# TimGyger/GPBoost

Measured on AMD Instinct MI355X. Metric: neg-log-lik + grad evals/sec, n=100k Vecchia m=30, higher is better.
Workload: dtype f64; 1 GPU; vecchia_gaussian_exact_lbfgs_unit; n=100000, num_neighbors=30, cov_function=exponential, ordering=random, parallelism=rows1

## Files before the change

gpboost_amd/csrc/vecchia_rows16.hip:

```cpp
#include <hip/hip_runtime.h>

#include <algorithm>
#include <type_traits>

#include "common.h"
#include "cov.h"
#include "kernels.h"

namespace gpb_amd {
namespace {

constexpr int kD3 = 3;

__device__ __forceinline__ void lds_sync() { asm volatile("s_waitcnt lgkmcnt(0)" ::: "memory"); }
__device__ __forceinline__ void cfence() { asm volatile("" ::: "memory"); }

template <int CTRL>
__device__ __forceinline__ double dpp32x2(double v) {
  const int lo = __builtin_amdgcn_mov_dpp(__double2loint(v), CTRL, 0xF, 0xF, true);
  const int hi = __builtin_amdgcn_mov_dpp(__double2hiint(v), CTRL, 0xF, 0xF, true);
  return __hiloint2double(hi, lo);
}

template <int L>
__device__ __forceinline__ double bcast16(double v) {
  const long b = __builtin_amdgcn_mov_dpp(__builtin_bit_cast(long, v), 0x150 + L, 0xF, 0xF, true);
  return __builtin_bit_cast(double, b);
}

template <int L, bool NOP = false>
__device__ __forceinline__ void fmac_bcast16(double& acc, double src, double mul) {
  if constexpr (NOP)
    asm volatile("s_nop 1\n\tv_fmac_f64_dpp %0, %1, %2 row_newbcast:%3 row_mask:0xf bank_mask:0xf"
                 : "+v"(acc)
                 : "v"(src), "v"(mul), "n"(L));
  else
    asm volatile("v_fmac_f64_dpp %0, %1, %2 row_newbcast:%3 row_mask:0xf bank_mask:0xf"
                 : "+v"(acc)
                 : "v"(src), "v"(mul), "n"(L));
}

__device__ __forceinline__ unsigned lds_addr(const double* p) {
  return (unsigned)(size_t)(const __attribute__((address_space(3))) double*)p;
}

template <int C>
__device__ __forceinline__ void lds_read_split2(double& a, double& b, unsigned up_a, unsigned up_b, unsigned lo_a,
                                                unsigned lo_b) {
  constexpr unsigned m16 = (0xFFFFu << C) & 0xFFFFu;
  constexpr unsigned long mask = m16 | m16 << 16;
  constexpr int CB = C + 16;
  unsigned long saved;
  asm volatile(
      "ds_read_b64 %0, %3 offset:%7\n\t"
      "ds_read_b64 %1, %4 offset:%8\n\t"
      "s_mov_b64 %2, exec\n\t"
      "s_and_b32 exec_lo, exec_lo, %11\n\t"
      "s_and_b32 exec_hi, exec_hi, %11\n\t"
      "ds_read_b64 %0, %5 offset:%9\n\t"
      "ds_read_b64 %1, %6 offset:%10\n\t"
      "s_mov_b64 exec, %2"
      : "=&v"(a), "=&v"(b), "=&s"(saved)
      : "v"(up_a), "v"(up_b), "v"(lo_a), "v"(lo_b), "n"(C * (C + 1) / 2 * 8), "n"(CB * (CB + 1) / 2 * 8), "n"(C * 8),
        "n"(CB * 8), "n"(mask)
      : "memory", "scc");
}

__device__ __forceinline__ double sum16(double v) {
  v += dpp32x2<0xB1>(v);
  v += dpp32x2<0x4E>(v);
  v += dpp32x2<0x141>(v);
  v += dpp32x2<0x140>(v);
  return v;
}

__device__ __forceinline__ double recip(double x) {
  double r = __builtin_amdgcn_rcp(x);
  r = fma(r, fma(-x, r, 1.), r);
  return fma(r, fma(-x, r, 1.), r);
}

template <int B, int E, class F>
__device__ __forceinline__ void sfor(F&& f) {
  if constexpr (B < E) {
    f(std::integral_constant<int, B>{});
    sfor<B + 1, E>(f);
  }
}

__device__ __forceinline__ int tri(int x) { return x * (x + 1) / 2; }

constexpr int kK = 32, kMK = 30;
constexpr int kPacked = kK * (kK + 1) / 2;

template <int CS>
constexpr int problem_doubles() { return kPacked + 48 * CS; }

typedef double v2d __attribute__((ext_vector_type(2)));


template <int ND>
__device__ __forceinline__ void load_points(const VecchiaRowsArgs& a, int d, int irow, int h, bool rv0, bool rv1,
                                            int nb0, int nb1, double (&xi)[ND], double (&x0)[ND], double (&x1)[ND]) {
#pragma unroll
  for (int q = 0; q < ND; ++q) {
    xi[q] = (q < d) ? a.X[(size_t)irow * d + q] : 0.;
    x0[q] = (q < d && rv0) ? a.X[(size_t)nb0 * d + q] : 0.;
    x1[q] = (q < d && rv1) ? a.X[(size_t)nb1 * d + q] : 0.;
  }
}

template <int ND>
__device__ __forceinline__ void pad_points(int h, bool rv0, bool rv1, const double (&xi)[ND], double (&x0)[ND],
                                           double (&x1)[ND]) {
  const int v1 = h + 16;
  const bool own1 = v1 == kMK;
#pragma unroll
  for (int q = 0; q < ND; ++q) x1[q] = own1 ? xi[q] : x1[q];
  x0[0] = rv0 ? x0[0] : 1e30 * (h + 1);
  x1[0] = (rv1 || own1) ? x1[0] : 1e30 * (v1 + 1);
}

template <int ND>
__device__ __forceinline__ void put_points(double* nbx, int h, const double (&x0)[ND], const double (&x1)[ND]) {
  const int v1 = h + 16;
#pragma unroll
  for (int q = 0; q < ND; ++q) {
    nbx[h * ND + q] = x0[q];
    nbx[(h + 31) * ND + q] = x0[q];
    if (v1 <= kMK) nbx[v1 * ND + q] = x1[q];
  }
}

template <int ND>
__device__ __forceinline__ double sq_dist(const double (&x)[ND], const double* xp) {
  double s = 0.;
#pragma unroll
  for (int q = 0; q < ND; ++q) {
    const double t = x[q] - xp[q];
    s += t * t;
  }
  return s;
}

constexpr int kDistRecs = 15 * 16;
static_assert(2 * kDistRecs == kRows16DistDoubles, "record layout");

template <int COV, int DIM, bool STORED>
__device__ __forceinline__ void rows16_body(const VecchiaRowsArgs& a) {
  constexpr int ND = DIM > 0 ? DIM : kD3;
  constexpr int CS = STORED ? 2 : ND;
  constexpr int PD = problem_doubles<CS>();
  static_assert(PD % 2 == 0, "16-byte aligned problems");
  extern __shared__ __attribute__((aligned(16))) double smem[];
  const int lane = threadIdx.x;
  const int g = lane >> 4;
  double* Cp = smem + g * PD;
  double* nbx = Cp + kPacked;
  const double var = a.var, phi = a.phi;
  const double cdiag = var * a.diag_mult + a.diag_add;
  const double delta = cdiag - var;
  const bool want_like = a.Y != nullptr;
  [[maybe_unused]] const int d = DIM > 0 ? DIM : a.d;

  double* acc = smem + 4 * PD + g * kVecchiaSums;
  if ((lane & 15) < kVecchiaSums) acc[lane & 15] = 0.;
  const int total = a.r1 - a.r0;
  const ExpCoef ek = ExpCoef::scalar();
  const int nsets = (total + 3) / 4, G = gridDim.x, w = blockIdx.x;
  const int R = (nsets + G - 1) / G, E = nsets - (R - 1) * G;
  int last_set = (R - 1) * G + w;
  if (a.sched == 1) {
    const long lo = (long)w * E / G, hi = (long)(w + 1) * E / G;
    last_set = hi > lo ? (R - 1) * G + (int)lo : nsets;
  }
  auto set_at = [&](int it) { return it + 1 < R ? it * G + w : last_set; };
  v2d rr[STORED ? 15 : 1];
  int pnb0 = 0, pnb1 = 0;
  auto prefetch = [&](int set) {
    if constexpr (STORED) {
      const int h = lane & 15;
      const int i = a.r0 + set * 4 + g;
      const bool active = i < a.r1;
      const int k = active ? min(i, a.m) : 0;
      pnb0 = h < k ? a.nbr[(size_t)(i - a.row_base) * a.m + h] : 0;
      pnb1 = h + 16 < k ? a.nbr[(size_t)(i - a.row_base) * a.m + h + 16] : 0;
      const v2d* rp = reinterpret_cast<const v2d*>(a.R) + (size_t)((active ? i : a.r0) - a.row_base) * kDistRecs + h;
#pragma unroll
      for (int q = 0; q < 15; ++q) rr[q] = rp[q * 16];
    }
  };
  if (set_at(0) < nsets) prefetch(set_at(0));
  for (int it = 0; it < R; ++it) {
    const int set = set_at(it);
    if (set >= nsets) break;
    const int base = set * 4;
    int h = lane & 15;
    asm volatile("" : "+v"(h));
    const int v1 = h + 16;
    const int i = a.r0 + base + g;
    const bool active = i < a.r1;
    const int k = active ? min(i, a.m) : 0;
    const bool rv0 = h < k, rv1 = v1 < k;
    const int irow = active ? i : a.r0;

    int nb0, nb1;
    double xi[ND], x0[ND], x1[ND];
    if constexpr (STORED) {
      nb0 = pnb0;
      nb1 = pnb1;
    } else {
      nb0 = rv0 ? a.nbr[(size_t)(i - a.row_base) * a.m + h] : 0;
      nb1 = rv1 ? a.nbr[(size_t)(i - a.row_base) * a.m + v1] : 0;
      load_points<ND>(a, d, irow, h, rv0, rv1, nb0, nb1, xi, x0, x1);
    }
    const double yi = want_like ? a.Y[irow] : 0.;
    double y0s = (want_like && rv0) ? a.Y[nb0] : 0.;
    double y1s = (want_like && rv1) ? a.Y[nb1] : 0.;
    if constexpr (!STORED) pad_points<ND>(h, rv0, rv1, xi, x0, x1);
    cfence();
    if constexpr (!STORED) put_points<ND>(nbx, h, x0, x1);
    Cp[tri(h) + h] = rv0 ? cdiag : 1.;
    Cp[tri(v1) + v1] = rv1 ? cdiag : 1.;
    lds_sync();

    double w0[15], w1[15];
    {
      const int b0 = tri(h) + h, b1 = tri(v1) + v1;
#pragma unroll
      for (int dl = 1; dl <= 15; ++dl) {
        double cv, dcv;
        if constexpr (STORED) cov_dcov_r<COV>(rr[dl - 1].x, var, phi, cv, dcv, ek);
        else cov_dcov_sq<COV>(sq_dist<ND>(x0, nbx + (h + dl) * CS), var, phi, cv, dcv, ek);
        Cp[b0 + h * dl + dl * (dl + 1) / 2] = cv;
        w0[dl - 1] = dcv;
      }
#pragma unroll
      for (int dl = 1; dl <= 15; ++dl) {
        double cv, dcv;
        if constexpr (STORED) cov_dcov_r<COV>(rr[dl - 1].y, var, phi, cv, dcv, ek);
        else cov_dcov_sq<COV>(sq_dist<ND>(x1, nbx + (v1 + dl) * CS), var, phi, cv, dcv, ek);
        const int pos = (v1 + dl <= kMK) ? b1 + v1 * dl + dl * (dl + 1) / 2 : b1 + dl - 31;
        Cp[pos] = cv;
        w1[dl - 1] = dcv;
      }
    }
    lds_sync();
    Cp[tri(kMK + 1) + h] = y0s;
    if (v1 < kMK) Cp[tri(kMK + 1) + v1] = y1s;
    else if (v1 == kMK) Cp[tri(kMK + 1) + kMK] = 0.;
    lds_sync();

    double r0[kK], r1[kK];
    {
      const unsigned lo0 = lds_addr(Cp + tri(h)), up0 = lds_addr(Cp + h);
      const unsigned lo1 = lds_addr(Cp + tri(v1)), up1 = lds_addr(Cp + v1);
      r0[0] = Cp[tri(h)];
#pragma unroll
      for (int c = 16; c < kK; ++c) r0[c] = Cp[tri(c) + h];
#pragma unroll
      for (int c = 0; c <= 16; ++c) r1[c] = Cp[tri(v1) + c];
      sfor<1, 16>([&](auto C) {
        constexpr int c = decltype(C)::value;
        double &p0 = r0[c], &p1 = r1[c + 16];
        lds_read_split2<c>(p0, p1, up0, up1, lo0, lo1);
      });
      sfor<0, 3>([&](auto Q) {
        constexpr int q = 1 + 5 * decltype(Q)::value;
        double &a0 = r0[q], &a1 = r0[q + 1], &a2 = r0[q + 2], &a3 = r0[q + 3], &a4 = r0[q + 4];
        double &b0 = r1[q + 16], &b1 = r1[q + 17], &b2 = r1[q + 18], &b3 = r1[q + 19], &b4 = r1[q + 20];
        if constexpr (q == 1)
          asm volatile("s_waitcnt lgkmcnt(0)" : "+v"(a0), "+v"(a1), "+v"(a2), "+v"(a3), "+v"(a4), "+v"(b0), "+v"(b1), "+v"(b2), "+v"(b3), "+v"(b4));
        else
          asm volatile("" : "+v"(a0), "+v"(a1), "+v"(a2), "+v"(a3), "+v"(a4), "+v"(b0), "+v"(b1), "+v"(b2), "+v"(b3), "+v"(b4));
      });
    }
    double c0, c1, dc0, dc1;
    cfence();
    {
      v2d* st = reinterpret_cast<v2d*>(__builtin_assume_aligned(nbx, 16)) + 2 * h;
      st[0] = v2d{r0[kMK], rv1 ? r1[kMK] : 0.};
      st[1] = v2d{y0s, y1s};
    }
#pragma unroll
    for (int dl = 1; dl <= 15; ++dl) {
      Cp[(dl - 1) * kK + h] = w0[dl - 1];
      Cp[(dl - 1) * kK + v1] = w1[dl - 1];
    }

    double dg0 = 1., dg1 = 1.;
    auto pivot = [&](auto J, double& m0, double& m1) {
      constexpr int j = decltype(J)::value;
      constexpr int jl = j & 15;
      const double piv = bcast16<jl>(j >= 16 ? r1[j] : r0[j]);
      const double rinv = recip(piv);
      const bool own = h == jl;
      const double f1 = r1[j] * rinv;
      if constexpr (j >= 16) {
        m0 = 0.;
        m1 = -(own ? 0. : f1);
        dg1 = own ? piv : dg1;
      } else {
        const double f0 = r0[j] * rinv;
        m0 = -(own ? 0. : f0);
        m1 = -f1;
        dg0 = own ? piv : dg0;
      }
    };
    sfor<0, kMK>([&](auto J) {
      constexpr int j = decltype(J)::value;
      constexpr bool jhi = j >= 16;
      double nf0, nf1;
      pivot(J, nf0, nf1);
      constexpr int cA = jhi ? 0 : 16;
      sfor<j + 1, kK>([&](auto C) {
        constexpr int c = decltype(C)::value;
        constexpr bool first = c == j + 1;
        const double& src = c >= 16 ? r1[j] : r0[j];
        if constexpr (c < cA) fmac_bcast16<c & 15, first>(r0[c], src, nf0);
        fmac_bcast16<c & 15, first && !(c < cA)>(r1[c], src, nf1);
      });
      sfor<j + 1, kK>([&](auto C) {
        constexpr int c = decltype(C)::value;
        double &p0 = r0[c], &p1 = r1[c];
        if constexpr (c < cA) asm volatile("" : "+v"(p0), "+v"(p1));
        else asm volatile("" : "+v"(p1));
      });
      if constexpr (!jhi) r0[j] = nf0;
    });
    {
      const double i1 = recip(dg1);
      const double na = rv1 ? -(r1[kMK] * i1) : 0., nw = rv1 ? -(r1[kMK + 1] * i1) : 0.;
      sfor<16, kMK>([&](auto C) {
        constexpr int c = decltype(C)::value;
        fmac_bcast16<c & 15, c == 16>(r0[kMK], na, r0[c]);
        fmac_bcast16<c & 15, c == 16>(r0[kMK + 1], nw, r0[c]);
      });
      sfor<0, 16>([&](auto J) {
        constexpr int j = decltype(J)::value;
        fmac_bcast16<j, true>(r0[kMK], r0[kMK], r0[j]);
        fmac_bcast16<j>(r0[kMK + 1], r0[kMK + 1], r0[j]);
      });
    }
    if constexpr (STORED) {
      cfence();
      const int nxt = it + 1 < R ? set_at(it + 1) : nsets;
      prefetch(nxt < nsets ? nxt : set);
    }
    {
      lds_sync();
      const v2d* st = reinterpret_cast<const v2d*>(__builtin_assume_aligned(nbx, 16)) + 2 * h;
      const v2d s0 = st[0], s1 = st[1];
      c0 = s0.x;
      c1 = s0.y;
      y0s = s1.x;
      y1s = s1.y;
      dc0 = Cp[h <= 14 ? h * kK + kMK : 14 * kK + 15];
      dc1 = h <= 13 ? Cp[(13 - h) * kK + v1] : 0.;
    }
    const double i0 = recip(dg0), i1 = recip(dg1);
    const double a0 = rv0 ? r0[kMK] * i0 : 0., w0v = rv0 ? r0[kMK + 1] * i0 : 0.;
    const double a1 = rv1 ? r1[kMK] * i1 : 0., w1v = rv1 ? r1[kMK + 1] * i1 : 0.;
    if (active && a.B_out != nullptr) {
      double* Bo = a.B_out + (size_t)(i - a.row_base) * a.m;
      if (h < a.m) Bo[h] = rv0 ? -a0 : 0.;
      if (v1 < a.m) Bo[v1] = rv1 ? -a1 : 0.;
    }

    double tA, tV;
    {
      v2d* av2 = reinterpret_cast<v2d*>(__builtin_assume_aligned(nbx, 16));
      cfence();
      av2[h] = v2d{a0, w0v};
      if (v1 <= kMK) av2[v1] = v2d{a1, w1v};
      av2[h + 31] = v2d{a0, w0v};
      lds_sync();
      double s10 = 0., s20 = 0., s11 = 0., s21 = 0.;
#pragma unroll
      for (int dl = 1; dl <= 15; ++dl) {
        const double wa = Cp[(dl - 1) * kK + h], wb = Cp[(dl - 1) * kK + v1];
        const v2d pa = av2[h + dl], pb = av2[v1 + dl];
        s10 = fma(wa, pa.x, s10);
        s20 = fma(wa, pa.y, s20);
        s11 = fma(wb, pb.x, s11);
        s21 = fma(wb, pb.y, s21);
      }
      tA = 2. * (a0 * s10 + a1 * s11);
      tV = w0v * s10 + a0 * s20 + w1v * s11 + a1 * s21;
    }

    const double ac = sum16(a0 * c0 + a1 * c1);
    const double ay = sum16(a0 * y0s + a1 * y1s);
    const double aa = sum16(a0 * a0 + a1 * a1);
    const double avv = sum16(a0 * w0v + a1 * w1v);
    const double dca = sum16(dc0 * a0 + dc1 * a1);
    const double dcv = sum16(dc0 * w0v + dc1 * w1v);
    const double ta = sum16(tA);
    const double tv = sum16(tV);
    const double D = var + a.d_nugget - ac;
    const double Dinv = 1. / D;
    if (active && h == 0 && a.Dinv_out != nullptr) a.Dinv_out[i - a.row_base] = Dinv;
    if (want_like && active && h == 0) {
      const double By = yi - ay;
      const double u = By * Dinv;
      const double dD_var = var - delta * aa - ac;
      const double uk_var = -delta * avv;
      const double dD_rng = -(2. * dca - ta);
      const double uk_rng = -(dcv - tv);
      acc[0] += log(D);
      acc[1] += By * u;
      acc[2] += uk_var * u - 0.5 * u * u * dD_var;
      acc[3] += uk_rng * u - 0.5 * u * u * dD_rng;
      acc[4] += Dinv * dD_var;
      acc[5] += Dinv * dD_rng;
    }
  }
  if (!want_like) return;
  __syncthreads();
  const double* red = smem + 4 * PD;
  if (lane < kVecchiaSums) {
    const double v = ((red[lane] + red[kVecchiaSums + lane]) + red[2 * kVecchiaSums + lane]) + red[3 * kVecchiaSums + lane];
    a.block_sums[(size_t)blockIdx.x * kVecchiaSums + lane] = v;
  }
}

template <int COV, int DIM>
__global__ void __launch_bounds__(64) __attribute__((amdgpu_waves_per_eu(2, 2))) vecchia_rows16_kernel(VecchiaRowsArgs a) {
  rows16_body<COV, DIM, false>(a);
}

template <int COV>
__global__ void __launch_bounds__(64) __attribute__((amdgpu_waves_per_eu(2, 2))) vecchia_rows16d_kernel(VecchiaRowsArgs a) {
  rows16_body<COV, 2, true>(a);
}

template <int DIM>
__global__ void __launch_bounds__(64) vecchia_rows16_dist_kernel(VecchiaRowsArgs a, double* R) {
  constexpr int ND = DIM > 0 ? DIM : kD3;
  extern __shared__ __attribute__((aligned(16))) double smem[];
  const int lane = threadIdx.x;
  const int g = lane >> 4, h = lane & 15, v1 = h + 16;
  double* nbx = smem + g * 48 * ND;
  const int d = DIM > 0 ? DIM : a.d;
  const int nsets = (a.r1 - a.r0 + 3) / 4;
  for (int set = blockIdx.x; set < nsets; set += gridDim.x) {
    const int i = a.r0 + set * 4 + g;
    const bool active = i < a.r1;
    const int k = active ? min(i, a.m) : 0;
    const bool rv0 = h < k, rv1 = v1 < k;
    const int irow = active ? i : a.r0;
    const int nb0 = rv0 ? a.nbr[(size_t)(i - a.row_base) * a.m + h] : 0;
    const int nb1 = rv1 ? a.nbr[(size_t)(i - a.row_base) * a.m + v1] : 0;
    double xi[ND], x0[ND], x1[ND];
    load_points<ND>(a, d, irow, h, rv0, rv1, nb0, nb1, xi, x0, x1);
    pad_points<ND>(h, rv0, rv1, xi, x0, x1);
    cfence();
    put_points<ND>(nbx, h, x0, x1);
    lds_sync();
    v2d* out = reinterpret_cast<v2d*>(R) + (size_t)(irow - a.row_base) * kDistRecs + h;
#pragma unroll
    for (int dl = 1; dl <= 15; ++dl) {
      const double ra = sqrt_nonneg(sq_dist<ND>(x0, nbx + (h + dl) * ND));
      const double rb = sqrt_nonneg(sq_dist<ND>(x1, nbx + (v1 + dl) * ND));
      if (active) out[(dl - 1) * 16] = v2d{ra, rb};
    }
  }
}

constexpr int kMaxGrid = 2048;

template <auto KERN>
int launch16_at(size_t lds, const VecchiaRowsArgs& a, hipStream_t s) {
  static int cap = 0;
  if (cap == 0) {
    int dev = 0, cus = 0, per_cu = 0;
    HIP_CHECK(hipGetDevice(&dev));
    HIP_CHECK(hipDeviceGetAttribute(&cus, hipDeviceAttributeMultiprocessorCount, dev));
    HIP_CHECK(hipOccupancyMaxActiveBlocksPerMultiprocessor(&per_cu, KERN, 64, lds));
    cap = std::max(1, std::min(per_cu * cus, kMaxGrid));
  }
  const int need = (a.r1 - a.r0 + 3) / 4;
  int blocks = std::min(need, cap);
  if (a.sched == 2) {
    const int rounds = (need + blocks - 1) / blocks;
    blocks = (need + rounds - 1) / rounds;
  }
  hipLaunchKernelGGL(KERN, dim3(blocks), dim3(64), lds, s, a);
  HIP_CHECK(hipGetLastError());
  return blocks;
}

template <int COV, int DIM>
int launch16(const VecchiaRowsArgs& a, hipStream_t s) {
  if (a.R != nullptr)
    return launch16_at<vecchia_rows16d_kernel<COV>>((size_t)(4 * problem_doubles<2>() + 4 * kVecchiaSums) * sizeof(double), a, s);
  constexpr int CS = DIM > 0 ? DIM : kD3;
  return launch16_at<vecchia_rows16_kernel<COV, DIM>>((size_t)(4 * problem_doubles<CS>() + 4 * kVecchiaSums) * sizeof(double), a, s);
}

}

int launch_vecchia_rows16(int cov_type, const VecchiaRowsArgs& a, hipStream_t s) {
  if (a.m > kMK) Fatal("16-lane row kernel: num_neighbors %d > %d", a.m, kMK);
  if (a.r1 <= a.r0) return 0;
  const bool planar = a.d == 2;
  switch (cov_type) {
    case kMatern05: return planar ? launch16<kMatern05, 2>(a, s) : launch16<kMatern05, 0>(a, s);
    case kMatern15: return planar ? launch16<kMatern15, 2>(a, s) : launch16<kMatern15, 0>(a, s);
    case kMatern25: return planar ? launch16<kMatern25, 2>(a, s) : launch16<kMatern25, 0>(a, s);
    case kGaussian: return planar ? launch16<kGaussian, 2>(a, s) : launch16<kGaussian, 0>(a, s);
    default: Fatal("unsupported covariance type %d", cov_type);
  }
  return 0;
}

void launch_vecchia_rows16_dist(const VecchiaRowsArgs& a, double* R, hipStream_t s) {
  if (a.m > kMK) Fatal("16-lane row kernel: num_neighbors %d > %d", a.m, kMK);
  if (a.d < 1 || a.d > kD3) Fatal("16-lane row kernel: dim_gp_coords %d", a.d);
  if (a.r1 <= a.r0) return;
  const int blocks = std::min((a.r1 - a.r0 + 3) / 4, 1 << 16);
  if (a.d == 2) hipLaunchKernelGGL(vecchia_rows16_dist_kernel<2>, dim3(blocks), dim3(64), 4 * 48 * 2 * sizeof(double), s, a, R);
  else hipLaunchKernelGGL(vecchia_rows16_dist_kernel<0>, dim3(blocks), dim3(64), 4 * 48 * kD3 * sizeof(double), s, a, R);
  HIP_CHECK(hipGetLastError());
}

}
```

Baseline: 6106 evals/s.

## Batch lane reductions, defer logs, and use exec-masked LDS writes in rows16 kernel

Replaces eight separate 16-lane DPP reductions with a combined transpose-and-add reduction that sums eight values in fewer DPP steps. Computes the pivot reciprocal once per pivot and stores it on the owning lane with exec-masked moves, so the later diagonal reciprocals are no longer needed. Covariance LDS writes now go through incremental addresses with constant offsets and exec-masked wrap writes, removing per-element index arithmetic and selects. log(D) is accumulated per lane across 16 iterations and reduced in a batch, cutting transcendental work by about 16x. Adds an environment override for grid size; the hand-written assembly and the changed reduction order carry correctness and rounding risk.

Result: faster. 6410 evals/s (median of 6 runs) (+5.0%).

```diff
diff --git a/gpboost_amd/csrc/vecchia_rows16.hip b/gpboost_amd/csrc/vecchia_rows16.hip
--- a/gpboost_amd/csrc/vecchia_rows16.hip
+++ b/gpboost_amd/csrc/vecchia_rows16.hip
@@ -1,6 +1,7 @@
 #include <hip/hip_runtime.h>
 
 #include <algorithm>
+#include <cstdlib>
 #include <type_traits>
 
 #include "common.h"
@@ -66,12 +67,79 @@
       : "memory", "scc");
 }
 
-__device__ __forceinline__ double sum16(double v) {
-  v += dpp32x2<0xB1>(v);
-  v += dpp32x2<0x4E>(v);
-  v += dpp32x2<0x141>(v);
-  v += dpp32x2<0x140>(v);
-  return v;
+constexpr unsigned rows2(unsigned m16) { return (m16 & 0xFFFFu) * 0x00010001u; }
+
+template <int J>
+__device__ __forceinline__ void own_lane(double& inv, double& mul, double rinv) {
+  unsigned long saved;
+  asm volatile(
+      "s_mov_b64 %2, exec\n\t"
+      "s_and_b32 exec_lo, %4, exec_lo\n\t"
+      "s_and_b32 exec_hi, %4, exec_hi\n\t"
+      "v_mov_b64 %0, %3\n\t"
+      "v_mov_b64 %1, 0\n\t"
+      "s_mov_b64 exec, %2"
+      : "+v"(inv), "+v"(mul), "=&s"(saved)
+      : "v"(rinv), "n"(rows2(1u << J))
+      : "scc");
+}
+
+template <int OFF>
+__device__ __forceinline__ void lds_write_at(unsigned addr, double v) {
+  asm volatile("ds_write_b64 %0, %1 offset:%2" : : "v"(addr), "v"(v), "n"(OFF) : "memory");
+}
+
+template <int DL>
+__device__ __forceinline__ void lds_write_wrap(unsigned in, unsigned wrap, double v) {
+  if constexpr (DL >= 15) {
+    lds_write_at<DL * 8>(wrap, v);
+  } else {
+    unsigned long saved;
+    asm volatile(
+        "s_mov_b64 %0, exec\n\t"
+        "s_and_b32 exec_lo, %4, exec_lo\n\t"
+        "s_and_b32 exec_hi, %4, exec_hi\n\t"
+        "ds_write_b64 %2, %3 offset:%6\n\t"
+        "s_andn2_b64 exec, %0, exec\n\t"
+        "ds_write_b64 %1, %3 offset:%5\n\t"
+        "s_mov_b64 exec, %0"
+        : "=&s"(saved)
+        : "v"(in), "v"(wrap), "v"(v), "n"(rows2(0xFFFFu << (15 - DL))), "n"(DL * (DL + 1) / 2 * 8), "n"(DL * 8)
+        : "memory", "scc");
+  }
+}
+
+template <int CTRL, int KEEP_X>
+__device__ __forceinline__ double pair_level(double x, double y) {
+  constexpr int KEEP_Y = 0xF & ~KEEP_X, SELF = 0xE4;
+  int plo = __builtin_amdgcn_mov_dpp(__double2loint(x), CTRL, 0xF, KEEP_X, false);
+  int phi = __builtin_amdgcn_mov_dpp(__double2hiint(x), CTRL, 0xF, KEEP_X, false);
+  plo = __builtin_amdgcn_update_dpp(plo, __double2loint(y), CTRL, 0xF, KEEP_Y, false);
+  phi = __builtin_amdgcn_update_dpp(phi, __double2hiint(y), CTRL, 0xF, KEEP_Y, false);
+  const int klo = __builtin_amdgcn_update_dpp(__double2loint(x), __double2loint(y), SELF, 0xF, KEEP_Y, false);
+  const int khi = __builtin_amdgcn_update_dpp(__double2hiint(x), __double2hiint(y), SELF, 0xF, KEEP_Y, false);
+  return __hiloint2double(khi, klo) + __hiloint2double(phi, plo);
+}
+
+__device__ __forceinline__ void sum16x8(const double (&q)[8], double (&t)[8]) {
+  double a[4], b[2];
+#pragma unroll
+  for (int k = 0; k < 4; ++k) a[k] = pair_level<0x140, 0x3>(q[2 * k], q[2 * k + 1]);
+#pragma unroll
+  for (int k = 0; k < 2; ++k) {
+    double v = pair_level<0x141, 0x5>(a[2 * k], a[2 * k + 1]);
+    v += dpp32x2<0xB1>(v);
+    v += dpp32x2<0x4E>(v);
+    b[k] = v;
+  }
+  t[0] = bcast16<0>(b[0]);
+  t[1] = bcast16<8>(b[0]);
+  t[2] = bcast16<4>(b[0]);
+  t[3] = bcast16<12>(b[0]);
+  t[4] = b[1];
+  t[5] = bcast16<8>(b[1]);
+  t[6] = bcast16<4>(b[1]);
+  t[7] = bcast16<12>(b[1]);
 }
 
 __device__ __forceinline__ double recip(double x) {
@@ -191,6 +259,16 @@
     }
   };
   if (set_at(0) < nsets) prefetch(set_at(0));
+  double keepD = 1.;
+  bool kept = false;
+  auto flush_logs = [&]() {
+    const double lg = log(keepD);
+    double s = acc[0];
+    sfor<0, 16>([&](auto L) { fmac_bcast16<decltype(L)::value, decltype(L)::value == 0>(s, lg, 1.); });
+    if ((lane & 15) == 0) acc[0] = s;
+    keepD = 1.;
+    kept = false;
+  };
   for (int it = 0; it < R; ++it) {
     const int set = set_at(it);
     if (set >= nsets) break;
@@ -227,23 +305,31 @@
     double w0[15], w1[15];
     {
       const int b0 = tri(h) + h, b1 = tri(v1) + v1;
-#pragma unroll
-      for (int dl = 1; dl <= 15; ++dl) {
+      const unsigned h8 = h * 8, v8 = v1 * 8;
+      unsigned p0 = lds_addr(Cp + b0), p1 = lds_addr(Cp + b1);
+      const unsigned pw = lds_addr(Cp + b1 - 31);
+      sfor<1, 16>([&](auto DL) {
+        constexpr int dl = decltype(DL)::value;
         double cv, dcv;
         if constexpr (STORED) cov_dcov_r<COV>(rr[dl - 1].x, var, phi, cv, dcv, ek);
         else cov_dcov_sq<COV>(sq_dist<ND>(x0, nbx + (h + dl) * CS), var, phi, cv, dcv, ek);
-        Cp[b0 + h * dl + dl * (dl + 1) / 2] = cv;
+        p0 += h8;
+        asm("" : "+v"(p0));
+        lds_write_at<dl * (dl + 1) / 2 * 8>(p0, cv);
         w0[dl - 1] = dcv;
-      }
-#pragma unroll
-      for (int dl = 1; dl <= 15; ++dl) {
+      });
+      sfor<1, 16>([&](auto DL) {
+        constexpr int dl = decltype(DL)::value;
         double cv, dcv;
         if constexpr (STORED) cov_dcov_r<COV>(rr[dl - 1].y, var, phi, cv, dcv, ek);
         else cov_dcov_sq<COV>(sq_dist<ND>(x1, nbx + (v1 + dl) * CS), var, phi, cv, dcv, ek);
-        const int pos = (v1 + dl <= kMK) ? b1 + v1 * dl + dl * (dl + 1) / 2 : b1 + dl - 31;
-        Cp[pos] = cv;
+        if constexpr (dl < 15) {
+          p1 += v8;
+          asm("" : "+v"(p1));
+        }
+        lds_write_wrap<dl>(p1, pw, cv);
         w1[dl - 1] = dcv;
-      }
+      });
     }
     lds_sync();
     Cp[tri(kMK + 1) + h] = y0s;
@@ -288,23 +374,19 @@
       Cp[(dl - 1) * kK + v1] = w1[dl - 1];
     }
 
-    double dg0 = 1., dg1 = 1.;
+    double i0 = 1., i1 = 1.;
     auto pivot = [&](auto J, double& m0, double& m1) {
       constexpr int j = decltype(J)::value;
       constexpr int jl = j & 15;
       const double piv = bcast16<jl>(j >= 16 ? r1[j] : r0[j]);
       const double rinv = recip(piv);
-      const bool own = h == jl;
-      const double f1 = r1[j] * rinv;
+      m1 = -(r1[j] * rinv);
       if constexpr (j >= 16) {
         m0 = 0.;
-        m1 = -(own ? 0. : f1);
-        dg1 = own ? piv : dg1;
+        own_lane<jl>(i1, m1, rinv);
       } else {
-        const double f0 = r0[j] * rinv;
-        m0 = -(own ? 0. : f0);
-        m1 = -f1;
-        dg0 = own ? piv : dg0;
+        m0 = -(r0[j] * rinv);
+        own_lane<jl>(i0, m0, rinv);
       }
     };
     sfor<0, kMK>([&](auto J) {
@@ -329,7 +411,6 @@
       if constexpr (!jhi) r0[j] = nf0;
     });
     {
-      const double i1 = recip(dg1);
       const double na = rv1 ? -(r1[kMK] * i1) : 0., nw = rv1 ? -(r1[kMK + 1] * i1) : 0.;
       sfor<16, kMK>([&](auto C) {
         constexpr int c = decltype(C)::value;
@@ -358,7 +439,6 @@
       dc0 = Cp[h <= 14 ? h * kK + kMK : 14 * kK + 15];
       dc1 = h <= 13 ? Cp[(13 - h) * kK + v1] : 0.;
     }
-    const double i0 = recip(dg0), i1 = recip(dg1);
     const double a0 = rv0 ? r0[kMK] * i0 : 0., w0v = rv0 ? r0[kMK + 1] * i0 : 0.;
     const double a1 = rv1 ? r1[kMK] * i1 : 0., w1v = rv1 ? r1[kMK + 1] * i1 : 0.;
     if (active && a.B_out != nullptr) {
@@ -389,14 +469,10 @@
       tV = w0v * s10 + a0 * s20 + w1v * s11 + a1 * s21;
     }
 
-    const double ac = sum16(a0 * c0 + a1 * c1);
-    const double ay = sum16(a0 * y0s + a1 * y1s);
-    const double aa = sum16(a0 * a0 + a1 * a1);
-    const double avv = sum16(a0 * w0v + a1 * w1v);
-    const double dca = sum16(dc0 * a0 + dc1 * a1);
-    const double dcv = sum16(dc0 * w0v + dc1 * w1v);
-    const double ta = sum16(tA);
-    const double tv = sum16(tV);
+    double gs[8];
+    sum16x8({a0 * c0 + a1 * c1, a0 * y0s + a1 * y1s, a0 * a0 + a1 * a1, a0 * w0v + a1 * w1v, dc0 * a0 + dc1 * a1,
+             dc0 * w0v + dc1 * w1v, tA, tV}, gs);
+    const double ac = gs[0], ay = gs[1], aa = gs[2], avv = gs[3], dca = gs[4], dcv = gs[5], ta = gs[6], tv = gs[7];
     const double D = var + a.d_nugget - ac;
     const double Dinv = 1. / D;
     if (active && h == 0 && a.Dinv_out != nullptr) a.Dinv_out[i - a.row_base] = Dinv;
@@ -407,15 +483,20 @@
       const double uk_var = -delta * avv;
       const double dD_rng = -(2. * dca - ta);
       const double uk_rng = -(dcv - tv);
-      acc[0] += log(D);
       acc[1] += By * u;
       acc[2] += uk_var * u - 0.5 * u * u * dD_var;
       acc[3] += uk_rng * u - 0.5 * u * u * dD_rng;
       acc[4] += Dinv * dD_var;
       acc[5] += Dinv * dD_rng;
     }
+    if (want_like) {
+      keepD = (active && h == (it & 15)) ? D : keepD;
+      kept = true;
+      if ((it & 15) == 15) flush_logs();
+    }
   }
   if (!want_like) return;
+  if (kept) flush_logs();
   __syncthreads();
   const double* red = smem + 4 * PD;
   if (lane < kVecchiaSums) {
@@ -481,6 +562,7 @@
   }
   const int need = (a.r1 - a.r0 + 3) / 4;
   int blocks = std::min(need, cap);
+  if (const char* e = std::getenv("GPBOOST_AMD_ROWS16_GRID")) blocks = std::min(blocks, std::max(1, std::atoi(e)));
   if (a.sched == 2) {
     const int rounds = (need + blocks - 1) / blocks;
     blocks = (need + rounds - 1) / rounds;
```
